# halajun/VDO_SLAM

Measured on AMD Instinct MI355X. Metric: frames/sec (per-frame hot path, KITTI-0000-shaped 1242x375) + ms/LM-iter (batch factor graph), higher is better.
Workload: dtype f64 (LM, RANSAC) / u8,i32,f32 (front-end, tracking)

## Files before the change

### include/vdo_slam_hip.h

```cpp
#ifndef VDO_SLAM_HIP_H_
#define VDO_SLAM_HIP_H_
#include <stdint.h>

#ifdef __cplusplus
extern "C" {
#endif

typedef enum vdo_status {
  VDO_OK = 0,
  VDO_ERR_INVALID = -1,
  VDO_ERR_NO_DEVICE = -2,
  VDO_ERR_OOM = -3,
  VDO_ERR_UNSUPPORTED = -4,
  VDO_ERR_INTERNAL = -5
} vdo_status;

int vdo_version(void);
const char* vdo_last_error(void);

typedef struct vdo_ctx vdo_ctx;
int vdo_ctx_create(int device, void* hip_stream, vdo_ctx** out);
int vdo_ctx_destroy(vdo_ctx* ctx);
int vdo_ctx_synchronize(vdo_ctx* ctx);
int vdo_ctx_stream(vdo_ctx* ctx, void** hip_stream_out);
// ... 174 lines not shown

typedef struct vdo_orb vdo_orb;
int vdo_orb_create(vdo_ctx* ctx, const vdo_orb_params* prm, int width, int height, vdo_orb** out);
int vdo_orb_destroy(vdo_orb* orb);
int vdo_orb_max_keypoints(const vdo_orb* orb, int* n);
int vdo_orb_extract(vdo_orb* orb, const uint8_t* gray, int stride, int src_is_device, vdo_keypoints* out);
int vdo_orb_extract_begin(vdo_orb* orb, const uint8_t* gray, int stride, int src_is_device);
int vdo_orb_extract_end(vdo_orb* orb, vdo_keypoints* out);
int vdo_orb_descriptors(vdo_orb* orb, uint8_t* desc32, int capacity_rows);
int vdo_orb_extract_desc(vdo_orb* orb, const uint8_t* gray, int stride, int src_is_device, vdo_keypoints* out, uint8_t* desc32);
int vdo_orb_level_info(vdo_orb* orb, int level, int* w, int* h, int* n_features, int* n_candidates);
int vdo_orb_get_pyramid(vdo_orb* orb, int level, uint8_t* out_bordered );
int vdo_orb_get_blurred(vdo_orb* orb, int level, uint8_t* out );
int vdo_orb_get_candidates(vdo_orb* orb, int level, float* x, float* y, float* response, float* angle, int cap, int* n);
int vdo_orb_last_timing(vdo_orb* orb, double ms[2]);
int vdo_orb_pyramid_launches(const vdo_orb* orb);

int vdo_depth_preprocess(vdo_ctx* ctx, float* depth, int64_t n, float bf, float depth_map_factor, int is_device);
int vdo_rgb2gray(vdo_ctx* ctx, const uint8_t* rgb, int64_t n_pixels, int channels, int rgb_order, uint8_t* gray);

typedef struct vdo_frame_images vdo_frame_images;
int vdo_frame_images_create(vdo_ctx* ctx, int width, int height, vdo_frame_images** out);
int vdo_frame_images_upload(vdo_frame_images* f, const float* depth, const float* flow, const int32_t* mask);
int vdo_frame_images_upload_on(vdo_ctx* ctx, vdo_frame_images* f, const float* depth, const float* flow, const int32_t* mask);
int vdo_frame_images_upload_device(vdo_frame_images* f, const float* depth_dev, const float* flow_dev, const int32_t* mask_dev);
int vdo_frame_images_depth_preprocess(vdo_frame_images* f, float bf, float depth_map_factor);
int vdo_frame_images_ingest_device(vdo_frame_images* f, const float* depth_dev, const float* flow_dev, const int32_t* mask_dev, float bf, float depth_map_factor,
                                   int convert_depth);
int vdo_frame_images_destroy(vdo_frame_images* f);
int vdo_frame_images_set_ctx(vdo_frame_images* f, vdo_ctx* ctx);
// ... 120 lines not shown
```

### vdo_slam_amd/csrc/orb.hip

```cpp
#include <algorithm>
#include <atomic>
#include <chrono>
#include <cmath>
#include <condition_variable>
#include <functional>
#include <memory>
#include <mutex>
#include <thread>
#include <cstring>
#include <vector>

#include "../../include/vdo_slam_hip.h"
#include "ctx.hpp"
#include "host_pool.hpp"
#include "orb_pattern.hpp"

namespace vdo {

constexpr int kEdge = 19, kHalfPatch = 15, kPatch = 31;
constexpr int kSpecCand = 24576;
constexpr int kMaxCellDim = 68;
static_assert(kMaxCellDim <= 128, "k_fast_cells packs cell-local coordinates in 7 bits");

struct LevelDesc { int w, h, bw, bh; int64_t off; int64_t off_inner; int64_t off_blur; };
struct CellDesc { int level, x0, y0, x1, y1, addx, addy, pad; };

__device__ __forceinline__ int reflect101(int p, int len) {
  if (len == 1) return 0;
  while (p < 0 || p >= len) { if (p < 0) p = -p; else p = 2 * (len - 1) - p; }
  return p;
}

__global__ void k_rgb2gray(const uint8_t* __restrict__ src, int64_t n, int ch, int rgb_order, uint8_t* __restrict__ dst) {
  const int64_t i = blockIdx.x * (int64_t)blockDim.x + threadIdx.x;
  if (i >= n) return;
// ... 142 lines not shown
  r[4] = c[3]; r[5] = c[-stride + 3]; r[6] = c[-2 * stride + 2]; r[7] = c[-3 * stride + 1];
  r[8] = c[-3 * stride]; r[9] = c[-3 * stride - 1]; r[10] = c[-2 * stride - 2]; r[11] = c[-stride - 3];
  r[12] = c[-3]; r[13] = c[stride - 3]; r[14] = c[2 * stride - 2]; r[15] = c[3 * stride - 1];
  int best = -1000;
#pragma unroll
  for (int s = 0; s < 16; ++s) {
    int mb = 1000, md = 1000;
#pragma unroll
    for (int k = 0; k < 9; ++k) { const int q = r[(s + k) & 15]; mb = min(mb, q - v); md = min(md, v - q); }
    best = max(best, max(mb, md));
  }
  return best > t ? best - 1 : 0;
}

__global__ __launch_bounds__(256) void k_fast_cells(const uint8_t* __restrict__ pyr, const LevelDesc* __restrict__ levels,
                                                    const CellDesc* __restrict__ cells, int ini_th, int min_th, int cell_cap,
                                                    int* __restrict__ out_cnt, uint32_t* __restrict__ out_pack) {
  __shared__ uint8_t roi[kMaxCellDim * kMaxCellDim];
  __shared__ uint8_t sc[kMaxCellDim * kMaxCellDim];
  __shared__ int s_wave[4], s_total;
  const CellDesc C = cells[blockIdx.x];
  const LevelDesc L = levels[C.level];
  const int w = C.x1 - C.x0, h = C.y1 - C.y0, tid = threadIdx.x;
  const uint8_t* img = pyr + L.off_inner;
  for (int i = tid; i < w * h; i += 256) { const int y = i / w, x = i - y * w; roi[y * kMaxCellDim + x] = img[(size_t)(C.y0 + y) * L.bw + (C.x0 + x)]; }
  __syncthreads();
  const int npix = w * h;
  const int per = (npix + 255) / 256;
  int t = ini_th;
  for (int pass = 0; pass < 2; ++pass) {
    for (int i = tid; i < npix; i += 256) {
      const int y = i / w, x = i - y * w;
      int s = 0;
      if (x >= 3 && x < w - 3 && y >= 3 && y < h - 3 && w >= 7 && h >= 7) s = fast_score_lds(roi, kMaxCellDim, x, y, t);
      sc[y * kMaxCellDim + x] = (uint8_t)s;
    }
// ... 14 lines not shown
    int incl = cnt;
#pragma unroll
    for (int off = 1; off < 64; off <<= 1) { const int v = __shfl_up(incl, off, 64); if (lane >= off) incl += v; }
    if (lane == 63) s_wave[wv] = incl;
    __syncthreads();
    if (tid == 0) { int a = 0; for (int q = 0; q < 4; ++q) { const int v = s_wave[q]; s_wave[q] = a; a += v; } s_total = a; }
    __syncthreads();
    const int total = s_total;
    if (total > 0 || pass == 1) {
      int pos = s_wave[wv] + incl - cnt;
      for (int k = 0; k < per; ++k) {
        if (!(keep & (1u << k))) continue;
        const int i = tid * per + k;
        const int y = i / w, x = i - y * w;
        if (pos < cell_cap)
          out_pack[(size_t)blockIdx.x * cell_cap + pos] = (uint32_t)x | ((uint32_t)y << 7) | ((uint32_t)sc[y * kMaxCellDim + x] << 24);
        ++pos;
      }
      if (tid == 0) out_cnt[blockIdx.x] = total;
      return;
    }
    t = min_th;
    __syncthreads();
  }
}

struct UMax { int v[kHalfPatch + 2]; };

__device__ __forceinline__ float fast_atan2_dev(float y, float x) {
  const float p1 = 0.9997878412794807f * (float)(180 / M_PI), p3 = -0.3258083974640975f * (float)(180 / M_PI);
  const float p5 = 0.1555786518463281f * (float)(180 / M_PI), p7 = -0.04432655554792128f * (float)(180 / M_PI);
  const float ax = fabsf(x), ay = fabsf(y);
  float a, c, c2;
  if (ax >= ay) { c = ay / (ax + (float)2.2204460492503131e-16); c2 = c * c; a = (((p7 * c2 + p5) * c2 + p3) * c2 + p1) * c; }
  else { c = ax / (ay + (float)2.2204460492503131e-16); c2 = c * c; a = 90.f - (((p7 * c2 + p5) * c2 + p3) * c2 + p1) * c; }
  if (x < 0) a = 180.f - a;
  if (y < 0) a = 360.f - a;
  return a;
}

__global__ __launch_bounds__(256) void k_compact_angle(const uint8_t* __restrict__ pyr, const LevelDesc* __restrict__ levels,
                                                       const CellDesc* __restrict__ cells, const int* __restrict__ cnt, const int* __restrict__ cell_level,
                                                       int* __restrict__ level_cnt, const uint32_t* __restrict__ pack, int ncells, int cell_cap, UMax um,
                                                       float* __restrict__ ox, float* __restrict__ oy, float* __restrict__ oresp,
                                                       float* __restrict__ oang, int* __restrict__ olevel) {
  const int cell = blockIdx.x;
  const int n = min(cnt[cell], cell_cap);
  const CellDesc C = cells[cell];
  const int lvl = C.level;
  const LevelDesc L = levels[lvl];
  const uint8_t* img = pyr + L.off_inner;
  const int lane = threadIdx.x & 63, wv = threadIdx.x >> 6;
  __shared__ int s_part[4], s_lvl[17];
// ... 7 lines not shown
    if (cell == 0 && threadIdx.x < 17) s_lvl[threadIdx.x] = 0;
    __syncthreads();
    base = s_part[0] + s_part[1] + s_part[2] + s_part[3];
    if (cell == 0) {
      int mx = 0;
      for (int c = threadIdx.x; c < ncells; c += 256) { const int r = cnt[c], v = min(r, cell_cap); if (v) atomicAdd(&s_lvl[cell_level[c]], v); mx = max(mx, r); }
      atomicMax(&s_lvl[16], mx);
      __syncthreads();
      if (threadIdx.x < 16) level_cnt[threadIdx.x] = s_lvl[threadIdx.x];
      if (threadIdx.x == 0) { int t = 0; for (int q = 0; q < 16; ++q) t += s_lvl[q]; level_cnt[16] = t; level_cnt[17] = s_lvl[16]; }
    }
  }
  for (int k = wv; k < n; k += 4) {
    const uint32_t pk = pack[(size_t)cell * cell_cap + k];
    const int x = (int)(pk & 0x7f) + C.addx, y = (int)((pk >> 7) & 0x7f) + C.addy, s = (int)(pk >> 24);
    const int cx = x + (kEdge - 3), cy = y + (kEdge - 3);
    int m10 = 0, m01 = 0;
    if (lane < 31) {
      const int v = lane - kHalfPatch;
      const int d = um.v[v < 0 ? -v : v];
      const uint8_t* row = img + (size_t)(cy + v) * L.bw + cx;
      int rs = 0;
      for (int u = -d; u <= d; ++u) { const int p = row[u]; m10 += u * p; rs += p; }
      m01 = v * rs;
    }
#pragma unroll
    for (int off = 32; off > 0; off >>= 1) { m10 += __shfl_down(m10, off, 64); m01 += __shfl_down(m01, off, 64); }
    if (lane == 0) {
      const int o = base + k;
      ox[o] = (float)x; oy[o] = (float)y; oresp[o] = (float)s; olevel[o] = lvl;
      oang[o] = fast_atan2_dev((float)m01, (float)m10);
    }
  }
}

struct Blur7 { int k[7]; };
struct OrbPattern { int4 q[64]; };

__device__ __forceinline__ void sincos_exact_dev(float angle, float* s_out, float* c_out) {
  const double x = (double)angle;
  const int k = (int)(x * 0.63661977236758138 + 0.5);
  const double r = (x - k * 1.57079632673412561417e+00) - k * 6.07710050650619224932e-11;
  const double z = r * r;
  const double sp = r * (1.0 + z * (-1.0 / 6 + z * (1.0 / 120 + z * (-1.0 / 5040 + z * (1.0 / 362880 + z * (-1.0 / 39916800 + z * (1.0 / 6227020800.0 +
                    z * (-1.0 / 1307674368000.0 + z * (1.0 / 355687428096000.0)))))))));
  const double cp = 1.0 + z * (-1.0 / 2 + z * (1.0 / 24 + z * (-1.0 / 720 + z * (1.0 / 40320 + z * (-1.0 / 3628800 + z * (1.0 / 479001600 +
                    z * (-1.0 / 87178291200.0 + z * (1.0 / 20922789888000.0))))))));
// ... 222 lines not shown
  std::vector<float> scale;
  UMax um{};
  Blur7 blur{};
  PyrDesc pyr{};
  PyrDesc pyr2{};
  std::vector<void*> allocs;
  uint8_t *d_src = nullptr, *d_pyr = nullptr, *d_blur = nullptr;
  LevelDesc* d_levels = nullptr; CellDesc* d_cells = nullptr; int* d_cell_level = nullptr;
  int *d_cnt = nullptr, *d_offs = nullptr, *d_level_cnt = nullptr; uint32_t* d_pack = nullptr;
  float *d_x = nullptr, *d_y = nullptr, *d_resp = nullptr, *d_ang = nullptr; int* d_lvl = nullptr;
  int64_t pyr_bytes = 0, blur_bytes = 0;
  int dense_cap = 0;
  std::vector<int> sel_dense;
  OrbPattern* d_pat = nullptr; int* d_sel = nullptr; uint8_t* d_desc = nullptr; int desc_cap = 0;
  float* h_pin = nullptr;
  float* h_over = nullptr; size_t h_over_n = 0;
  const float *hx = nullptr, *hy = nullptr, *hresp = nullptr, *hang = nullptr; std::vector<int> hlevel_cnt;
  int n_cand = 0;
  QuadTree qt[16];
  std::vector<int> sel[16];
  std::unique_ptr<LevelPool> pool;
  double ms_device = 0, ms_tree = 0;
  bool begun = false;
  hipEvent_t ev_cand = nullptr;
  std::chrono::steady_clock::time_point t_begin;
};

extern "C" int vdo_orb_pyramid_launches(const vdo_orb* o) {
  if (!o) return set_error(VDO_ERR_INVALID, "null handle");
  return o->pyr.n_levels ? (o->pyr2.lv1 > o->pyr2.lv0 ? 2 : 1) : (int)o->levels.size();
// ... 126 lines not shown
        for (int axis = 0; axis < 2; ++axis) {
          const int len = axis ? D->h[l] : D->w[l];
          for (int t0 = 0; t0 < len; t0 += 32) {
            int d0 = t0, d1 = std::min(t0 + 31, len - 1);
            for (int k = l; k > D->base; --k) {
              int s0, s1;
              src_range(d0, d1, axis ? D->sy[k] : D->sx[k], axis ? D->h[k - 1] : D->w[k - 1], axis == 1, s0, s1);
              d0 = s0; d1 = s1;
              worst = std::max(worst, d1 - d0 + 1);
            }
          }
        }
      }
    }
    if (worst > kPyrRegion) P.n_levels = 0;
  }
  {
    int* umax = o->um.v;
    int v, v0;
    const int vmax = (int)std::floor(kHalfPatch * std::sqrt(2.f) / 2 + 1);
    const int vmin = (int)std::ceil(kHalfPatch * std::sqrt(2.f) / 2);
    const double hp2 = kHalfPatch * kHalfPatch;
    for (v = 0; v <= vmax; ++v) umax[v] = (int)lrint(std::sqrt(hp2 - v * v));
    for (v = kHalfPatch, v0 = 0; v >= vmin; --v) { while (umax[v0] == umax[v0 + 1]) ++v0; umax[v] = v0; ++v0; }
  }
  {
    double kd[7], sum = 0;
    for (int i = 0; i < 7; ++i) { const double x = i - 3; kd[i] = std::exp(-0.5 / 4.0 * x * x); sum += kd[i]; }
    for (int i = 0; i < 7; ++i) o->blur.k[i] = (int)lrint((double)(float)(kd[i] / sum) * 256);
  }
  hipStream_t s = ctx->stream;
  auto dev = [&](size_t bytes) -> void* { void* p = nullptr; if (hipMalloc(&p, bytes ? bytes : 8) != hipSuccess) return nullptr; o->allocs.push_back(p); return p; };
  o->dense_cap = o->ncells * o->cell_cap;
  o->d_src = (uint8_t*)dev((size_t)w * h * 4);
  o->d_pyr = (uint8_t*)dev(o->pyr_bytes); o->d_blur = (uint8_t*)dev(o->blur_bytes);
  o->d_levels = (LevelDesc*)dev(sizeof(LevelDesc) * NL); o->d_cells = (CellDesc*)dev(sizeof(CellDesc) * o->ncells);
  o->d_cell_level = (int*)dev(4 * (size_t)o->ncells);
  o->d_pat = (OrbPattern*)dev(sizeof(OrbPattern));
  o->d_cnt = (int*)dev(4 * (size_t)o->ncells); o->d_offs = (int*)dev(4 * ((size_t)o->ncells + 1)); o->d_level_cnt = (int*)dev(4 * 32);
  o->d_pack = (uint32_t*)dev(4 * (size_t)o->dense_cap);
  o->d_x = (float*)dev(4 * (size_t)o->dense_cap * 5);
  if (o->d_x) {
    o->d_y = o->d_x + (size_t)o->dense_cap; o->d_resp = o->d_x + 2 * (size_t)o->dense_cap; o->d_ang = o->d_x + 3 * (size_t)o->dense_cap;
    o->d_lvl = (int*)(o->d_x + 4 * (size_t)o->dense_cap);
  }
  if (hipHostMalloc((void**)&o->h_pin, 4 * (32 + 5 * (size_t)kSpecCand)) != hipSuccess) o->h_pin = nullptr;
  for (void* p : o->allocs) if (!p) { vdo_orb_destroy(o); return set_error(VDO_ERR_OOM, "hipMalloc failed"); }
  if (!o->d_lvl || !o->h_pin) { vdo_orb_destroy(o); return set_error(VDO_ERR_OOM, "hipMalloc failed"); }
  hipMemcpyAsync(o->d_levels, o->levels.data(), sizeof(LevelDesc) * NL, hipMemcpyHostToDevice, s);
  hipMemcpyAsync(o->d_cells, o->cells.data(), sizeof(CellDesc) * o->ncells, hipMemcpyHostToDevice, s);
  hipMemcpyAsync(o->d_cell_level, o->cell_level.data(), 4 * (size_t)o->ncells, hipMemcpyHostToDevice, s);
  static_assert(sizeof(kOrbPattern31) == sizeof(OrbPattern), "256 tests x 4 signed bytes");
  hipMemcpyAsync(o->d_pat, kOrbPattern31, sizeof(OrbPattern), hipMemcpyHostToDevice, s);
  if (hipStreamSynchronize(s) != hipSuccess) { vdo_orb_destroy(o); return set_error(VDO_ERR_NO_DEVICE, "orb upload failed"); }
  if (hipEventCreateWithFlags(&o->ev_cand, hipEventDisableTiming) != hipSuccess) { vdo_orb_destroy(o); return set_error(VDO_ERR_NO_DEVICE, "hipEventCreate failed"); }
  {
    const char* e = std::getenv("VDO_ORB_THREADS");
    const int nw = e ? std::atoi(e) : 3;
    if (nw > 0) o->pool.reset(new LevelPool(std::min(nw, 15)));
  }
  *out = o;
// ... 10 lines not shown
      const LevelDesc& B = o->levels[o->pyr2.base];
      hipLaunchKernelGGL(k_pyramid_all, dim3(o->pyr2.tile_off[o->pyr2.n_levels]), dim3(256), 0, s, (const uint8_t*)(o->d_pyr + B.off_inner), B.bw, o->pyr2, (const LevelDesc*)o->d_levels, o->d_pyr);
    }
  } else {
    {
      const LevelDesc& L = o->levels[0];
      hipLaunchKernelGGL(k_border_copy, dim3((L.bw + 31) / 32, (L.bh + 7) / 8), tb, 0, s, gray_dev, L.w, L.h, stride, o->d_pyr + L.off, L.bw, L.bh);
    }
    for (int l = 1; l < NL; ++l) {
      const LevelDesc &P = o->levels[l - 1], &L = o->levels[l];
      const double sx = 1. / ((double)L.w / P.w), sy = 1. / ((double)L.h / P.h);
      hipLaunchKernelGGL(k_resize_border, dim3((L.bw + 31) / 32, (L.bh + 7) / 8), tb, 0, s, (const uint8_t*)(o->d_pyr + P.off_inner), P.w, P.h, P.bw,
                         o->d_pyr + L.off, L.w, L.h, sx, sy);
    }
  }
  hipLaunchKernelGGL(k_fast_cells, dim3(o->ncells), dim3(256), 0, s, (const uint8_t*)o->d_pyr, (const LevelDesc*)o->d_levels, (const CellDesc*)o->d_cells,
                     o->prm.ini_th, o->prm.min_th, o->cell_cap, o->d_cnt, o->d_pack);
  hipLaunchKernelGGL(k_compact_angle, dim3(o->ncells), dim3(256), 0, s, (const uint8_t*)o->d_pyr, (const LevelDesc*)o->d_levels, (const CellDesc*)o->d_cells,
                     (const int*)o->d_cnt, (const int*)o->d_cell_level, o->d_level_cnt, (const uint32_t*)o->d_pack, o->ncells, o->cell_cap, o->um, o->d_x, o->d_y, o->d_resp, o->d_ang, o->d_lvl);
  return VDO_OK;
}

static void orb_blur_stage(vdo_orb* o) {
  hipStream_t s = o->ctx->stream;
  BlurTiles bt{};
  int tot = 0;
  for (int l = 0; l < o->prm.n_levels; ++l) {
    const LevelDesc& L = o->levels[l];
    bt.off[l] = tot; bt.tiles_x[l] = (L.w + 31) / 32;
    tot += bt.tiles_x[l] * ((L.h + 31) / 32);
  }
  bt.off[o->prm.n_levels] = tot;
  hipLaunchKernelGGL(k_blur7_all, dim3(tot), dim3(256), 0, s, (const uint8_t*)o->d_pyr, (const LevelDesc*)o->d_levels, o->prm.n_levels, bt, o->blur, o->d_blur);
}

extern "C" int vdo_orb_extract_begin(vdo_orb* o, const uint8_t* gray, int stride, int src_is_device) {
  if (!o || !gray) return set_error(VDO_ERR_INVALID, "vdo_orb_extract_begin: null argument");
  int rc = ctx_bind(o->ctx);
  if (rc != VDO_OK) return rc;
  hipStream_t s = o->ctx->stream;
  const uint8_t* src = gray;
  int sstride = stride;
  if (!src_is_device) {
    if (stride == o->w) hipMemcpyAsync(o->d_src, gray, (size_t)o->w * o->h, hipMemcpyHostToDevice, s);
    else hipMemcpy2DAsync(o->d_src, o->w, gray, stride, o->w, o->h, hipMemcpyHostToDevice, s);
    src = o->d_src; sstride = o->w;
  }
  o->t_begin = std::chrono::steady_clock::now();
  orb_device_stage(o, src, sstride);
  int* hdr = (int*)o->h_pin;
  float* rows = o->h_pin + 32;
  const int spec = std::min(kSpecCand, o->dense_cap);
  hipMemcpyAsync(hdr, o->d_level_cnt, 4 * 32, hipMemcpyDeviceToHost, s);
  hipMemcpy2DAsync(rows, 4 * (size_t)spec, o->d_x, 4 * (size_t)o->dense_cap, 4 * (size_t)spec, 5, hipMemcpyDeviceToHost, s);
  hipEventRecord(o->ev_cand, s);
  orb_blur_stage(o);
  o->begun = true;
  return VDO_OK;
}

extern "C" int vdo_orb_extract(vdo_orb* o, const uint8_t* gray, int stride, int src_is_device, vdo_keypoints* out) {
  int rc = vdo_orb_extract_begin(o, gray, stride, src_is_device);
  return rc != VDO_OK ? rc : vdo_orb_extract_end(o, out);
}

extern "C" int vdo_orb_extract_end(vdo_orb* o, vdo_keypoints* out) {
  if (!o || !out) return set_error(VDO_ERR_INVALID, "vdo_orb_extract_end: null argument");
  if (!o->begun) return set_error(VDO_ERR_INVALID, "vdo_orb_extract_end without vdo_orb_extract_begin");
  o->begun = false;
  int rc = ctx_bind(o->ctx);
  if (rc != VDO_OK) return rc;
  hipStream_t s = o->ctx->stream;
  const auto t_begin = o->t_begin;
  int* hdr = (int*)o->h_pin;
  float* rows = o->h_pin + 32;
  const int spec = std::min(kSpecCand, o->dense_cap);
  if (hipEventSynchronize(o->ev_cand) != hipSuccess) return set_error(VDO_ERR_NO_DEVICE, "orb device stage failed: %s", hipGetErrorString(hipGetLastError()));
  if (hdr[17] > o->cell_cap) {
    o->hlevel_cnt.clear(); o->sel_dense.clear();
    return set_error(VDO_ERR_UNSUPPORTED, "vdo_orb_extract: a FAST cell has %d candidates, more than the %d kept per cell", hdr[17], o->cell_cap);
  }
  const int total = hdr[16];
  o->n_cand = total;
  o->hlevel_cnt.assign(hdr, hdr + 16);
  size_t pitch = (size_t)spec;
  if (total > spec) {
    if (o->h_over_n < (size_t)total) {
      if (o->h_over) hipHostFree(o->h_over);
      o->h_over = nullptr; o->h_over_n = 0;
      if (hipHostMalloc((void**)&o->h_over, 4 * 5 * (size_t)total) != hipSuccess) return set_error(VDO_ERR_OOM, "hipHostMalloc failed");
      o->h_over_n = (size_t)total;
    }
    hipMemcpy2DAsync(o->h_over, 4 * (size_t)total, o->d_x, 4 * (size_t)o->dense_cap, 4 * (size_t)total, 5, hipMemcpyDeviceToHost, s);
    if (hipStreamSynchronize(s) != hipSuccess) return set_error(VDO_ERR_NO_DEVICE, "orb D2H failed");
    rows = o->h_over; pitch = (size_t)total;
  }
  o->hx = rows; o->hy = rows + pitch; o->hresp = rows + 2 * pitch; o->hang = rows + 3 * pitch;
  const auto t_dev = std::chrono::steady_clock::now();
  const int NL = o->prm.n_levels;
  int lvl_pos[17];
  lvl_pos[0] = 0;
  for (int l = 0; l < NL; ++l) lvl_pos[l + 1] = lvl_pos[l] + o->hlevel_cnt[l];
  const int minB = kEdge - 3;
  auto level_task = [&](int l) {
    const LevelDesc& L = o->levels[l];
    const int pos = lvl_pos[l];
    o->qt[l].run(o->hx + pos, o->hy + pos, o->hresp + pos, o->hlevel_cnt[l], minB, L.w - kEdge + 3, minB, L.h - kEdge + 3, o->nfeat[l], o->sel[l]);
  };
  if (o->pool) o->pool->run(NL, level_task);
  else for (int l = 0; l < NL; ++l) level_task(l);
  int n = 0;
  o->sel_dense.clear();
  for (int l = 0; l < NL; ++l) {
    const int pos = lvl_pos[l];
    const float *cx = o->hx + pos, *cy = o->hy + pos, *cr = o->hresp + pos, *ca = o->hang + pos;
    const int patch = (int)(kPatch * o->scale[l]);
    for (int id : o->sel[l]) {
      o->sel_dense.push_back(pos + id);
      if (n >= out->capacity) return set_error(VDO_ERR_INVALID, "vdo_orb_extract: keypoint capacity %d too small", out->capacity);
      float x = cx[id] + minB, y = cy[id] + minB;
      if (l != 0) { x = x * o->scale[l]; y = y * o->scale[l]; }
      out->x[n] = x; out->y[n] = y; out->response[n] = cr[id]; out->angle[n] = ca[id];
      out->octave[n] = l; out->size[n] = (float)patch;
      ++n;
    }
  }
  out->n = n;
  const auto t_end = std::chrono::steady_clock::now();
  o->ms_device = std::chrono::duration<double, std::milli>(t_dev - t_begin).count();
  o->ms_tree = std::chrono::duration<double, std::milli>(t_end - t_dev).count();
  return VDO_OK;
}

extern "C" int vdo_orb_descriptors(vdo_orb* o, uint8_t* desc32, int capacity_rows) {
  if (!o || !desc32) return set_error(VDO_ERR_INVALID, "vdo_orb_descriptors: null argument");
  const int n = (int)o->sel_dense.size();
  if (n > capacity_rows) return set_error(VDO_ERR_INVALID, "vdo_orb_descriptors: %d keypoints, room for %d", n, capacity_rows);
  if (n == 0) return VDO_OK;
  int rc = ctx_bind(o->ctx);
  if (rc != VDO_OK) return rc;
  hipStream_t s = o->ctx->stream;
  if (n > o->desc_cap) {
    const int cap = std::max(n, 4096);
    int* ns = nullptr; uint8_t* nd = nullptr;
    if (hipMalloc((void**)&ns, 4 * (size_t)cap) != hipSuccess || hipMalloc((void**)&nd, 32 * (size_t)cap) != hipSuccess) { if (ns) hipFree(ns); return set_error(VDO_ERR_OOM, "hipMalloc failed"); }
// ... 11 lines not shown
  return VDO_OK;
}

extern "C" int vdo_orb_extract_desc(vdo_orb* o, const uint8_t* gray, int stride, int src_is_device, vdo_keypoints* out, uint8_t* desc32) {
  int rc = vdo_orb_extract(o, gray, stride, src_is_device, out);
  if (rc != VDO_OK || !desc32) return rc;
  return vdo_orb_descriptors(o, desc32, out->capacity);
}

extern "C" int vdo_orb_last_timing(vdo_orb* o, double ms[2]) {
  if (!o || !ms) return set_error(VDO_ERR_INVALID, "null argument");
  ms[0] = o->ms_device; ms[1] = o->ms_tree;
  return VDO_OK;
}

extern "C" int vdo_orb_level_info(vdo_orb* o, int level, int* w, int* h, int* n_features, int* n_candidates) {
  if (!o || level < 0 || level >= o->prm.n_levels) return set_error(VDO_ERR_INVALID, "bad level");
  if (w) *w = o->levels[level].w;
  if (h) *h = o->levels[level].h;
  if (n_features) *n_features = o->nfeat[level];
  if (n_candidates) *n_candidates = o->hlevel_cnt.empty() ? 0 : o->hlevel_cnt[level];
  return VDO_OK;
}

extern "C" int vdo_orb_get_pyramid(vdo_orb* o, int level, uint8_t* out_bordered) {
  if (!o || !out_bordered || level < 0 || level >= o->prm.n_levels) return set_error(VDO_ERR_INVALID, "bad argument");
  int rc = ctx_bind(o->ctx);
  if (rc != VDO_OK) return rc;
  const LevelDesc& L = o->levels[level];
  if (hipMemcpy(out_bordered, o->d_pyr + L.off, (size_t)L.bw * L.bh, hipMemcpyDeviceToHost) != hipSuccess) return set_error(VDO_ERR_NO_DEVICE, "D2H failed");
// ... 67 lines not shown
```

### vdo_slam_amd/frontend.py

```python
from __future__ import annotations

import ctypes as C

import numpy as np

from . import _capi as K


class OrbParamsC(C.Structure):
    _fields_ = [("n_features", C.c_int32), ("scale_factor", C.c_float), ("n_levels", C.c_int32),
                ("ini_th", C.c_int32), ("min_th", C.c_int32)]


class KeypointsC(C.Structure):
    _fields_ = [("capacity", C.c_int32), ("n", C.c_int32), ("x", K.c_float_p), ("y", K.c_float_p),
                ("response", K.c_float_p), ("angle", K.c_float_p), ("size", K.c_float_p), ("octave", K.c_int32_p)]


def _fp(a): return a.ctypes.data_as(K.c_float_p)
def _ip(a): return a.ctypes.data_as(K.c_int32_p)
def _u8(a): return a.ctypes.data_as(K.c_uint8_p)


_declared = False
# ... 76 lines not shown
            st = self._dev_out = (cap, a, octave, kp, C.byref(kp), _lib().vdo_orb_extract)
        _, a, octave, kp, kp_ref, fn = st
        K.check(fn(self._h, C.cast(C.c_void_p(gray_ptr), K.c_uint8_p), stride, 1, kp_ref))
        n = kp.n
        out = {k: v[:n] for k, v in a.items()}
        out["octave"] = octave[:n]
        return out

    def last_timing(self):
        ms = (C.c_double * 2)()
        L = _lib()
        L.vdo_orb_last_timing.argtypes = [C.c_void_p, C.POINTER(C.c_double)]
        K.check(L.vdo_orb_last_timing(self._h, ms))
        return ms[0], ms[1]

    def pyramid_launches(self):
        L = _lib()
        L.vdo_orb_pyramid_launches.argtypes = [C.c_void_p]
        return int(L.vdo_orb_pyramid_launches(self._h))

    def level_info(self, level):
        w, h, nf, nc = C.c_int(), C.c_int(), C.c_int(), C.c_int()
        K.check(_lib().vdo_orb_level_info(self._h, level, C.byref(w), C.byref(h), C.byref(nf), C.byref(nc)))
        return w.value, h.value, nf.value, nc.value

    def pyramid(self, level):
        w, h, _, _ = self.level_info(level)
        out = np.zeros((h + 38, w + 38), np.uint8)
        K.check(_lib().vdo_orb_get_pyramid(self._h, level, _u8(out)))
        return out
# ... 141 lines not shown
```

Baseline: 1388.

## Pipeline ORB per level group so host quadtrees overlap device FAST work

Splits pyramid construction, FAST detection and compaction into up to three level groups. Each group publishes its candidates straight into mapped pinned host memory along with a ticket word, and host worker threads spin on that word and start the per-level quadtree distribution as soon as their group is ready. Orientation is computed in a separate pass afterwards. The aim is to hide host quadtree time behind the remaining device work instead of waiting for the whole device stage to finish. In exchange it adds host busy-wait spinning, system-scope fences, extra small single-block launches, and a fallback path when candidate counts overflow.

```diff
diff --git a/include/vdo_slam_hip.h b/include/vdo_slam_hip.h
--- a/include/vdo_slam_hip.h
+++ b/include/vdo_slam_hip.h
@@ -212,6 +212,7 @@
 int vdo_orb_get_blurred(vdo_orb* orb, int level, uint8_t* out );
 int vdo_orb_get_candidates(vdo_orb* orb, int level, float* x, float* y, float* response, float* angle, int cap, int* n);
 int vdo_orb_last_timing(vdo_orb* orb, double ms[2]);
+int vdo_orb_last_level_timing(vdo_orb* orb, double group_ms[5], double level_ms[16]);
 int vdo_orb_pyramid_launches(const vdo_orb* orb);
 
 int vdo_depth_preprocess(vdo_ctx* ctx, float* depth, int64_t n, float bf, float depth_map_factor, int is_device);
diff --git a/vdo_slam_amd/csrc/orb.hip b/vdo_slam_amd/csrc/orb.hip
--- a/vdo_slam_amd/csrc/orb.hip
+++ b/vdo_slam_amd/csrc/orb.hip
@@ -19,6 +19,8 @@
 
 constexpr int kEdge = 19, kHalfPatch = 15, kPatch = 31;
 constexpr int kSpecCand = 24576;
+constexpr int kMaxGroups = 3;
+constexpr int kPinHdr = 32 + 32 * 4;
 constexpr int kMaxCellDim = 68;
 static_assert(kMaxCellDim <= 128, "k_fast_cells packs cell-local coordinates in 7 bits");
 
@@ -191,12 +193,13 @@
 }
 
 __global__ __launch_bounds__(256) void k_fast_cells(const uint8_t* __restrict__ pyr, const LevelDesc* __restrict__ levels,
-                                                    const CellDesc* __restrict__ cells, int ini_th, int min_th, int cell_cap,
+                                                    const CellDesc* __restrict__ cells, int cell0, int ini_th, int min_th, int cell_cap,
                                                     int* __restrict__ out_cnt, uint32_t* __restrict__ out_pack) {
   __shared__ uint8_t roi[kMaxCellDim * kMaxCellDim];
   __shared__ uint8_t sc[kMaxCellDim * kMaxCellDim];
   __shared__ int s_wave[4], s_total;
-  const CellDesc C = cells[blockIdx.x];
+  const int cell = cell0 + blockIdx.x;
+  const CellDesc C = cells[cell];
   const LevelDesc L = levels[C.level];
   const int w = C.x1 - C.x0, h = C.y1 - C.y0, tid = threadIdx.x;
   const uint8_t* img = pyr + L.off_inner;
@@ -241,10 +244,10 @@
         const int i = tid * per + k;
         const int y = i / w, x = i - y * w;
         if (pos < cell_cap)
-          out_pack[(size_t)blockIdx.x * cell_cap + pos] = (uint32_t)x | ((uint32_t)y << 7) | ((uint32_t)sc[y * kMaxCellDim + x] << 24);
+          out_pack[(size_t)cell * cell_cap + pos] = (uint32_t)x | ((uint32_t)y << 7) | ((uint32_t)sc[y * kMaxCellDim + x] << 24);
         ++pos;
       }
-      if (tid == 0) out_cnt[blockIdx.x] = total;
+      if (tid == 0) out_cnt[cell] = total;
       return;
     }
     t = min_th;
@@ -264,6 +267,21 @@
   if (x < 0) a = 180.f - a;
   if (y < 0) a = 360.f - a;
   return a;
+}
+
+__device__ __forceinline__ float ic_angle_wave(const uint8_t* __restrict__ img, int bw, int cx, int cy, int lane, const UMax& um) {
+  int m10 = 0, m01 = 0;
+  if (lane < 31) {
+    const int v = lane - kHalfPatch;
+    const int d = um.v[v < 0 ? -v : v];
+    const uint8_t* row = img + (size_t)(cy + v) * bw + cx;
+    int rs = 0;
+    for (int u = -d; u <= d; ++u) { const int p = row[u]; m10 += u * p; rs += p; }
+    m01 = v * rs;
+  }
+#pragma unroll
+  for (int off = 32; off > 0; off >>= 1) { m10 += __shfl_down(m10, off, 64); m01 += __shfl_down(m01, off, 64); }
+  return fast_atan2_dev((float)m01, (float)m10);
 }
 
 __global__ __launch_bounds__(256) void k_compact_angle(const uint8_t* __restrict__ pyr, const LevelDesc* __restrict__ levels,
@@ -301,23 +319,84 @@
   for (int k = wv; k < n; k += 4) {
     const uint32_t pk = pack[(size_t)cell * cell_cap + k];
     const int x = (int)(pk & 0x7f) + C.addx, y = (int)((pk >> 7) & 0x7f) + C.addy, s = (int)(pk >> 24);
-    const int cx = x + (kEdge - 3), cy = y + (kEdge - 3);
-    int m10 = 0, m01 = 0;
-    if (lane < 31) {
-      const int v = lane - kHalfPatch;
-      const int d = um.v[v < 0 ? -v : v];
-      const uint8_t* row = img + (size_t)(cy + v) * L.bw + cx;
-      int rs = 0;
-      for (int u = -d; u <= d; ++u) { const int p = row[u]; m10 += u * p; rs += p; }
-      m01 = v * rs;
-    }
-#pragma unroll
-    for (int off = 32; off > 0; off >>= 1) { m10 += __shfl_down(m10, off, 64); m01 += __shfl_down(m01, off, 64); }
+    const float ang = ic_angle_wave(img, L.bw, x + (kEdge - 3), y + (kEdge - 3), lane, um);
     if (lane == 0) {
       const int o = base + k;
       ox[o] = (float)x; oy[o] = (float)y; oresp[o] = (float)s; olevel[o] = lvl;
-      oang[o] = fast_atan2_dev((float)m01, (float)m10);
-    }
+      oang[o] = ang;
+    }
+  }
+}
+
+__global__ __launch_bounds__(256) void k_compact_group(const CellDesc* __restrict__ cells, const int* __restrict__ cnt, const uint32_t* __restrict__ pack, int c0, int cell_cap,
+                                                       int* __restrict__ cell_off, float* __restrict__ ox, float* __restrict__ oy, float* __restrict__ oresp, int* __restrict__ olevel) {
+  __shared__ int s_part[4];
+  const int cell = c0 + blockIdx.x;
+  const int lane = threadIdx.x & 63, wv = threadIdx.x >> 6;
+  int a = 0;
+  for (int c = threadIdx.x; c < cell; c += 256) a += min(cnt[c], cell_cap);
+#pragma unroll
+  for (int off = 32; off > 0; off >>= 1) a += __shfl_down(a, off, 64);
+  if (lane == 0) s_part[wv] = a;
+  __syncthreads();
+  const int base = s_part[0] + s_part[1] + s_part[2] + s_part[3];
+  const int n = min(cnt[cell], cell_cap);
+  const CellDesc C = cells[cell];
+  if (threadIdx.x == 0) cell_off[cell] = base;
+  for (int k = threadIdx.x; k < n; k += 256) {
+    const uint32_t pk = pack[(size_t)cell * cell_cap + k];
+    const int o = base + k;
+    ox[o] = (float)((int)(pk & 0x7f) + C.addx); oy[o] = (float)((int)((pk >> 7) & 0x7f) + C.addy); oresp[o] = (float)(int)(pk >> 24); olevel[o] = C.level;
+  }
+}
+
+constexpr int kPublishThreads = 1024;
+__global__ __launch_bounds__(kPublishThreads) void k_publish(const int* __restrict__ cnt, const int* __restrict__ cell_level, int c0, int c1, int cell_cap, int spec,
+                                                             const float* __restrict__ src, size_t spitch, int nrows, float* __restrict__ dst, size_t dpitch,
+                                                             int* __restrict__ hdr, uint32_t ticket) {
+  __shared__ int s_lvl[19];
+  const int tid = threadIdx.x;
+  if (tid < 19) s_lvl[tid] = 0;
+  __syncthreads();
+  int before = 0, tot = 0, mx = 0;
+  for (int c = tid; c < c1; c += kPublishThreads) {
+    const int r = cnt[c], v = min(r, cell_cap);
+    if (c < c0) before += v;
+    else { tot += v; if (v) atomicAdd(&s_lvl[cell_level[c]], v); mx = max(mx, r); }
+  }
+#pragma unroll
+  for (int off = 32; off > 0; off >>= 1) { before += __shfl_down(before, off, 64); tot += __shfl_down(tot, off, 64); mx = max(mx, __shfl_down(mx, off, 64)); }
+  if ((tid & 63) == 0) { atomicAdd(&s_lvl[18], before); atomicAdd(&s_lvl[16], tot); atomicMax(&s_lvl[17], mx); }
+  __syncthreads();
+  const int base = s_lvl[18], n = max(0, min(base + s_lvl[16], spec) - base);
+  if (tid < 18) hdr[tid] = tid == 16 ? base + s_lvl[16] : s_lvl[tid];
+  for (int e0 = tid; e0 < nrows * n; e0 += 8 * kPublishThreads) {
+    float v[8];
+#pragma unroll
+    for (int u = 0; u < 8; ++u) { const int e = e0 + u * kPublishThreads; if (e < nrows * n) { const int r = e / n, i = e - r * n; v[u] = src[r * spitch + base + i]; } }
+#pragma unroll
+    for (int u = 0; u < 8; ++u) { const int e = e0 + u * kPublishThreads; if (e < nrows * n) { const int r = e / n, i = e - r * n; dst[r * dpitch + base + i] = v[u]; } }
+  }
+  __threadfence_system();
+  __syncthreads();
+  if (tid == 0) *(volatile uint32_t*)(hdr + 18) = ticket;
+}
+
+__global__ __launch_bounds__(256) void k_angle_all(const uint8_t* __restrict__ pyr, const LevelDesc* __restrict__ levels, const CellDesc* __restrict__ cells,
+                                                   const int* __restrict__ cnt, const int* __restrict__ cell_off, const uint32_t* __restrict__ pack, int cell_cap, UMax um,
+                                                   float* __restrict__ oang) {
+  const int cell = blockIdx.x;
+  const int n = min(cnt[cell], cell_cap);
+  if (n == 0) return;
+  const CellDesc C = cells[cell];
+  const LevelDesc L = levels[C.level];
+  const uint8_t* img = pyr + L.off_inner;
+  const int lane = threadIdx.x & 63, wv = threadIdx.x >> 6, base = cell_off[cell];
+  for (int k = wv; k < n; k += 4) {
+    const uint32_t pk = pack[(size_t)cell * cell_cap + k];
+    const int x = (int)(pk & 0x7f) + C.addx, y = (int)((pk >> 7) & 0x7f) + C.addy;
+    const float ang = ic_angle_wave(img, L.bw, x + (kEdge - 3), y + (kEdge - 3), lane, um);
+    if (lane == 0) oang[base + k] = ang;
   }
 }
 
@@ -570,6 +649,13 @@
   std::vector<int> sel_dense;
   OrbPattern* d_pat = nullptr; int* d_sel = nullptr; uint8_t* d_desc = nullptr; int desc_cap = 0;
   float* h_pin = nullptr;
+  float* h_pin_dev = nullptr;
+  PyrDesc pyr1{};
+  int n_groups = 0, grp_lvl[kMaxGroups + 1] = {}, grp_cell[kMaxGroups + 1] = {};
+  uint32_t seq = 0;
+  bool piped = false;
+  const uint8_t* pend_gray = nullptr; int pend_stride = 0, pend_dev = 0;
+  double ms_group[kMaxGroups + 2] = {}, ms_level[16] = {};
   float* h_over = nullptr; size_t h_over_n = 0;
   const float *hx = nullptr, *hy = nullptr, *hresp = nullptr, *hang = nullptr; std::vector<int> hlevel_cnt;
   int n_cand = 0;
@@ -726,6 +812,21 @@
       }
     }
     if (worst > kPyrRegion) P.n_levels = 0;
+    if (P.n_levels) {
+      int* gl = o->grp_lvl;
+      gl[0] = 0; gl[1] = 1; o->n_groups = 1;
+      if (NL > 1) { gl[2] = split + 1; o->n_groups = 2; }
+      if (NL > split + 1) { gl[3] = NL; o->n_groups = 3; }
+      for (int g = 0; g <= o->n_groups; ++g)
+        o->grp_cell[g] = (int)(std::lower_bound(o->cell_level.begin(), o->cell_level.end(), gl[g]) - o->cell_level.begin());
+      PyrDesc& P1 = o->pyr1;
+      P1 = P;
+      P1.lv0 = 1;
+      int tot = 0;
+      for (int l = 0; l <= NL; ++l) P1.tile_off[l] = 0;
+      for (int l = P1.lv0; l < P1.lv1; ++l) { P1.tile_off[l] = tot; tot += P1.tiles_x[l] * ((P1.h[l] + 31) / 32); }
+      for (int l = std::max(P1.lv1, P1.lv0); l <= NL; ++l) P1.tile_off[l] = tot;
+    }
   }
   {
     int* umax = o->um.v;
@@ -756,7 +857,13 @@
     o->d_y = o->d_x + (size_t)o->dense_cap; o->d_resp = o->d_x + 2 * (size_t)o->dense_cap; o->d_ang = o->d_x + 3 * (size_t)o->dense_cap;
     o->d_lvl = (int*)(o->d_x + 4 * (size_t)o->dense_cap);
   }
-  if (hipHostMalloc((void**)&o->h_pin, 4 * (32 + 5 * (size_t)kSpecCand)) != hipSuccess) o->h_pin = nullptr;
+  if (hipHostMalloc((void**)&o->h_pin, 4 * (kPinHdr + 5 * (size_t)kSpecCand), hipHostMallocMapped) != hipSuccess) o->h_pin = nullptr;
+  if (o->h_pin) {
+    std::memset(o->h_pin, 0, 4 * (size_t)kPinHdr);
+    void* dp = nullptr;
+    if (hipHostGetDevicePointer(&dp, o->h_pin, 0) == hipSuccess) o->h_pin_dev = (float*)dp;
+    else { (void)hipGetLastError(); o->n_groups = 0; }
+  }
   for (void* p : o->allocs) if (!p) { vdo_orb_destroy(o); return set_error(VDO_ERR_OOM, "hipMalloc failed"); }
   if (!o->d_lvl || !o->h_pin) { vdo_orb_destroy(o); return set_error(VDO_ERR_OOM, "hipMalloc failed"); }
   hipMemcpyAsync(o->d_levels, o->levels.data(), sizeof(LevelDesc) * NL, hipMemcpyHostToDevice, s);
@@ -797,11 +904,43 @@
                          o->d_pyr + L.off, L.w, L.h, sx, sy);
     }
   }
-  hipLaunchKernelGGL(k_fast_cells, dim3(o->ncells), dim3(256), 0, s, (const uint8_t*)o->d_pyr, (const LevelDesc*)o->d_levels, (const CellDesc*)o->d_cells,
+  hipLaunchKernelGGL(k_fast_cells, dim3(o->ncells), dim3(256), 0, s, (const uint8_t*)o->d_pyr, (const LevelDesc*)o->d_levels, (const CellDesc*)o->d_cells, 0,
                      o->prm.ini_th, o->prm.min_th, o->cell_cap, o->d_cnt, o->d_pack);
   hipLaunchKernelGGL(k_compact_angle, dim3(o->ncells), dim3(256), 0, s, (const uint8_t*)o->d_pyr, (const LevelDesc*)o->d_levels, (const CellDesc*)o->d_cells,
                      (const int*)o->d_cnt, (const int*)o->d_cell_level, o->d_level_cnt, (const uint32_t*)o->d_pack, o->ncells, o->cell_cap, o->um, o->d_x, o->d_y, o->d_resp, o->d_ang, o->d_lvl);
   return VDO_OK;
+}
+
+static void orb_device_stage_groups(vdo_orb* o, const uint8_t* gray_dev, int stride) {
+  hipStream_t s = o->ctx->stream;
+  const int spec = std::min(kSpecCand, o->dense_cap);
+  int* ghdr = (int*)o->h_pin_dev + 32;
+  float* hrows = o->h_pin_dev + kPinHdr;
+  for (int g = 0; g < o->n_groups; ++g) {
+    if (g == 0) {
+      const LevelDesc& L = o->levels[0];
+      hipLaunchKernelGGL(k_border_copy, dim3((L.bw + 31) / 32, (L.bh + 7) / 8), dim3(32, 8), 0, s, gray_dev, L.w, L.h, stride, o->d_pyr + L.off, L.bw, L.bh);
+    } else if (g == 1) {
+      hipLaunchKernelGGL(k_pyramid_all, dim3(o->pyr1.tile_off[o->pyr1.n_levels]), dim3(256), 0, s, gray_dev, stride, o->pyr1, (const LevelDesc*)o->d_levels, o->d_pyr);
+    } else {
+      const LevelDesc& B = o->levels[o->pyr2.base];
+      hipLaunchKernelGGL(k_pyramid_all, dim3(o->pyr2.tile_off[o->pyr2.n_levels]), dim3(256), 0, s, (const uint8_t*)(o->d_pyr + B.off_inner), B.bw, o->pyr2, (const LevelDesc*)o->d_levels, o->d_pyr);
+    }
+    const int c0 = o->grp_cell[g], c1 = o->grp_cell[g + 1];
+    if (c1 > c0)
+      hipLaunchKernelGGL(k_fast_cells, dim3(c1 - c0), dim3(256), 0, s, (const uint8_t*)o->d_pyr, (const LevelDesc*)o->d_levels, (const CellDesc*)o->d_cells, c0,
+                         o->prm.ini_th, o->prm.min_th, o->cell_cap, o->d_cnt, o->d_pack);
+    if (c1 > c0)
+      hipLaunchKernelGGL(k_compact_group, dim3(c1 - c0), dim3(256), 0, s, (const CellDesc*)o->d_cells, (const int*)o->d_cnt, (const uint32_t*)o->d_pack, c0, o->cell_cap,
+                         o->d_offs, o->d_x, o->d_y, o->d_resp, o->d_lvl);
+    hipLaunchKernelGGL(k_publish, dim3(1), dim3(kPublishThreads), 0, s, (const int*)o->d_cnt, (const int*)o->d_cell_level, c0, c1, o->cell_cap, spec,
+                       (const float*)o->d_x, (size_t)o->dense_cap, 3, hrows, (size_t)spec, ghdr + 32 * g, o->seq);
+  }
+  if (o->ncells)
+    hipLaunchKernelGGL(k_angle_all, dim3(o->ncells), dim3(256), 0, s, (const uint8_t*)o->d_pyr, (const LevelDesc*)o->d_levels, (const CellDesc*)o->d_cells,
+                       (const int*)o->d_cnt, (const int*)o->d_offs, (const uint32_t*)o->d_pack, o->cell_cap, o->um, o->d_ang);
+  hipLaunchKernelGGL(k_publish, dim3(1), dim3(kPublishThreads), 0, s, (const int*)o->d_cnt, (const int*)o->d_cell_level, 0, o->ncells, o->cell_cap, spec,
+                     (const float*)o->d_ang, (size_t)o->dense_cap, 1, hrows + 3 * (size_t)spec, (size_t)spec, ghdr + 32 * kMaxGroups, o->seq);
 }
 
 static void orb_blur_stage(vdo_orb* o) {
@@ -817,10 +956,17 @@
   hipLaunchKernelGGL(k_blur7_all, dim3(tot), dim3(256), 0, s, (const uint8_t*)o->d_pyr, (const LevelDesc*)o->d_levels, o->prm.n_levels, bt, o->blur, o->d_blur);
 }
 
-extern "C" int vdo_orb_extract_begin(vdo_orb* o, const uint8_t* gray, int stride, int src_is_device) {
+static int orb_begin_prepare(vdo_orb* o, const uint8_t* gray) {
   if (!o || !gray) return set_error(VDO_ERR_INVALID, "vdo_orb_extract_begin: null argument");
   int rc = ctx_bind(o->ctx);
   if (rc != VDO_OK) return rc;
+  o->t_begin = std::chrono::steady_clock::now();
+  o->piped = o->n_groups > 0 && !std::getenv("VDO_ORB_NO_LEVEL_PIPELINE");
+  if (o->piped && ++o->seq == 0) ++o->seq;
+  return VDO_OK;
+}
+
+static void orb_begin_launch(vdo_orb* o, const uint8_t* gray, int stride, int src_is_device) {
   hipStream_t s = o->ctx->stream;
   const uint8_t* src = gray;
   int sstride = stride;
@@ -829,22 +975,89 @@
     else hipMemcpy2DAsync(o->d_src, o->w, gray, stride, o->w, o->h, hipMemcpyHostToDevice, s);
     src = o->d_src; sstride = o->w;
   }
-  o->t_begin = std::chrono::steady_clock::now();
-  orb_device_stage(o, src, sstride);
-  int* hdr = (int*)o->h_pin;
-  float* rows = o->h_pin + 32;
-  const int spec = std::min(kSpecCand, o->dense_cap);
-  hipMemcpyAsync(hdr, o->d_level_cnt, 4 * 32, hipMemcpyDeviceToHost, s);
-  hipMemcpy2DAsync(rows, 4 * (size_t)spec, o->d_x, 4 * (size_t)o->dense_cap, 4 * (size_t)spec, 5, hipMemcpyDeviceToHost, s);
+  if (o->piped) {
+    orb_device_stage_groups(o, src, sstride);
+  } else {
+    orb_device_stage(o, src, sstride);
+    int* hdr = (int*)o->h_pin;
+    float* rows = o->h_pin + kPinHdr;
+    const int spec = std::min(kSpecCand, o->dense_cap);
+    hipMemcpyAsync(hdr, o->d_level_cnt, 4 * 32, hipMemcpyDeviceToHost, s);
+    hipMemcpy2DAsync(rows, 4 * (size_t)spec, o->d_x, 4 * (size_t)o->dense_cap, 4 * (size_t)spec, 5, hipMemcpyDeviceToHost, s);
+  }
   hipEventRecord(o->ev_cand, s);
   orb_blur_stage(o);
+  o->ms_group[kMaxGroups + 1] = std::chrono::duration<double, std::milli>(std::chrono::steady_clock::now() - o->t_begin).count();
+}
+
+extern "C" int vdo_orb_extract_begin(vdo_orb* o, const uint8_t* gray, int stride, int src_is_device) {
+  int rc = orb_begin_prepare(o, gray);
+  if (rc != VDO_OK) return rc;
+  orb_begin_launch(o, gray, stride, src_is_device);
   o->begun = true;
   return VDO_OK;
 }
 
 extern "C" int vdo_orb_extract(vdo_orb* o, const uint8_t* gray, int stride, int src_is_device, vdo_keypoints* out) {
-  int rc = vdo_orb_extract_begin(o, gray, stride, src_is_device);
-  return rc != VDO_OK ? rc : vdo_orb_extract_end(o, out);
+  int rc = orb_begin_prepare(o, gray);
+  if (rc != VDO_OK) return rc;
+  if (o->piped && o->pool && out) { o->pend_gray = gray; o->pend_stride = stride; o->pend_dev = src_is_device; }
+  else orb_begin_launch(o, gray, stride, src_is_device);
+  o->begun = true;
+  return vdo_orb_extract_end(o, out);
+}
+
+static bool orb_trees_by_group(vdo_orb* o) {
+  const int NL = o->prm.n_levels, G = o->n_groups, spec = std::min(kSpecCand, o->dense_cap), minB = kEdge - 3;
+  const int* ghdr = (const int*)o->h_pin + 32;
+  const float* rows = o->h_pin + kPinHdr;
+  const auto t_begin = o->t_begin;
+  std::atomic<int> bad{0};
+  double seen[16];
+  auto wait_group = [&](int g) {
+    const int* hdr = ghdr + 32 * g;
+    volatile const uint32_t* word = (volatile const uint32_t*)(hdr + 18);
+    const auto t0 = std::chrono::steady_clock::now();
+    for (uint32_t spins = 0; *word != o->seq; ++spins) {
+      if (bad.load(std::memory_order_relaxed)) return false;
+      if ((spins & 1023u) == 1023u && std::chrono::duration<double, std::milli>(std::chrono::steady_clock::now() - t0).count() > 200.0) { bad.store(1); return false; }
+      __builtin_ia32_pause();
+    }
+    std::atomic_thread_fence(std::memory_order_acquire);
+    if (g < kMaxGroups && (hdr[17] > o->cell_cap || hdr[16] > spec)) { bad.store(1); return false; }
+    return true;
+  };
+  auto level_task = [&](int l) {
+    int g = 0;
+    while (l >= o->grp_lvl[g + 1]) ++g;
+    if (!wait_group(g)) return;
+    const auto t0 = std::chrono::steady_clock::now();
+    const int* hdr = ghdr + 32 * g;
+    int pos = hdr[16];
+    for (int k = o->grp_lvl[g + 1] - 1; k >= l; --k) pos -= hdr[k];
+    const LevelDesc& L = o->levels[l];
+    o->hlevel_cnt[l] = hdr[l];
+    o->qt[l].run(rows + pos, rows + spec + pos, rows + 2 * (size_t)spec + pos, hdr[l], minB, L.w - kEdge + 3, minB, L.h - kEdge + 3, o->nfeat[l], o->sel[l]);
+    const auto t1 = std::chrono::steady_clock::now();
+    seen[l] = std::chrono::duration<double, std::milli>(t0 - t_begin).count();
+    o->ms_level[l] = std::chrono::duration<double, std::milli>(t1 - t0).count();
+  };
+  for (int l = 0; l < 16; ++l) { seen[l] = 0; o->ms_level[l] = 0; }
+  o->hlevel_cnt.assign(16, 0);
+  auto mine = [&] {
+    if (o->pend_gray) { const uint8_t* g = o->pend_gray; o->pend_gray = nullptr; orb_begin_launch(o, g, o->pend_stride, o->pend_dev); }
+    level_task(0);
+  };
+  if (o->pool) o->pool->run_beside(NL - 1, [&](int i) { level_task(i + 1); }, mine);
+  else for (int l = 0; l < NL; ++l) level_task(l);
+  for (int g = 0; g < G; ++g) {
+    double m = 0;
+    for (int l = o->grp_lvl[g]; l < o->grp_lvl[g + 1]; ++l) if (seen[l] > 0 && (m == 0 || seen[l] < m)) m = seen[l];
+    o->ms_group[g] = m;
+  }
+  if (bad.load() || !wait_group(kMaxGroups)) return false;
+  o->ms_group[kMaxGroups] = std::chrono::duration<double, std::milli>(std::chrono::steady_clock::now() - t_begin).count();
+  return true;
 }
 
 extern "C" int vdo_orb_extract_end(vdo_orb* o, vdo_keypoints* out) {
@@ -852,13 +1065,26 @@
   if (!o->begun) return set_error(VDO_ERR_INVALID, "vdo_orb_extract_end without vdo_orb_extract_begin");
   o->begun = false;
   int rc = ctx_bind(o->ctx);
-  if (rc != VDO_OK) return rc;
+  if (rc != VDO_OK) { o->pend_gray = nullptr; return rc; }
   hipStream_t s = o->ctx->stream;
   const auto t_begin = o->t_begin;
+  const int NL = o->prm.n_levels;
   int* hdr = (int*)o->h_pin;
-  float* rows = o->h_pin + 32;
+  float* rows = o->h_pin + kPinHdr;
   const int spec = std::min(kSpecCand, o->dense_cap);
-  if (hipEventSynchronize(o->ev_cand) != hipSuccess) return set_error(VDO_ERR_NO_DEVICE, "orb device stage failed: %s", hipGetErrorString(hipGetLastError()));
+  int lvl_pos[17];
+  bool trees_done = false;
+  for (int g = 0; g <= kMaxGroups; ++g) o->ms_group[g] = 0;
+  if (o->piped) trees_done = orb_trees_by_group(o);
+  if (!trees_done && hipEventSynchronize(o->ev_cand) != hipSuccess) { o->hlevel_cnt.clear(); o->sel_dense.clear(); return set_error(VDO_ERR_NO_DEVICE, "orb device stage failed: %s", hipGetErrorString(hipGetLastError())); }
+  if (o->piped) {
+    const int* ghdr = (const int*)o->h_pin + 32;
+    for (int k = 0; k < 32; ++k) hdr[k] = 0;
+    for (int g = 0; g < o->n_groups; ++g) {
+      for (int l = o->grp_lvl[g]; l < o->grp_lvl[g + 1]; ++l) hdr[l] = ghdr[32 * g + l];
+      hdr[16] = ghdr[32 * g + 16]; hdr[17] = std::max(hdr[17], ghdr[32 * g + 17]);
+    }
+  }
   if (hdr[17] > o->cell_cap) {
     o->hlevel_cnt.clear(); o->sel_dense.clear();
     return set_error(VDO_ERR_UNSUPPORTED, "vdo_orb_extract: a FAST cell has %d candidates, more than the %d kept per cell", hdr[17], o->cell_cap);
@@ -868,6 +1094,7 @@
   o->hlevel_cnt.assign(hdr, hdr + 16);
   size_t pitch = (size_t)spec;
   if (total > spec) {
+    trees_done = false;
     if (o->h_over_n < (size_t)total) {
       if (o->h_over) hipHostFree(o->h_over);
       o->h_over = nullptr; o->h_over_n = 0;
@@ -880,19 +1107,22 @@
   }
   o->hx = rows; o->hy = rows + pitch; o->hresp = rows + 2 * pitch; o->hang = rows + 3 * pitch;
   const auto t_dev = std::chrono::steady_clock::now();
-  const int NL = o->prm.n_levels;
-  int lvl_pos[17];
   lvl_pos[0] = 0;
   for (int l = 0; l < NL; ++l) lvl_pos[l + 1] = lvl_pos[l] + o->hlevel_cnt[l];
+  if (!trees_done) {
+    const int minB = kEdge - 3;
+    auto level_task = [&](int l) {
+      const auto t0 = std::chrono::steady_clock::now();
+      const LevelDesc& L = o->levels[l];
+      const int pos = lvl_pos[l];
+      o->qt[l].run(o->hx + pos, o->hy + pos, o->hresp + pos, o->hlevel_cnt[l], minB, L.w - kEdge + 3, minB, L.h - kEdge + 3, o->nfeat[l], o->sel[l]);
+      o->ms_level[l] = std::chrono::duration<double, std::milli>(std::chrono::steady_clock::now() - t0).count();
+    };
+    if (o->pool) o->pool->run(NL, level_task);
+    else for (int l = 0; l < NL; ++l) level_task(l);
+  }
+  int n = 0;
   const int minB = kEdge - 3;
-  auto level_task = [&](int l) {
-    const LevelDesc& L = o->levels[l];
-    const int pos = lvl_pos[l];
-    o->qt[l].run(o->hx + pos, o->hy + pos, o->hresp + pos, o->hlevel_cnt[l], minB, L.w - kEdge + 3, minB, L.h - kEdge + 3, o->nfeat[l], o->sel[l]);
-  };
-  if (o->pool) o->pool->run(NL, level_task);
-  else for (int l = 0; l < NL; ++l) level_task(l);
-  int n = 0;
   o->sel_dense.clear();
   for (int l = 0; l < NL; ++l) {
     const int pos = lvl_pos[l];
@@ -910,8 +1140,8 @@
   }
   out->n = n;
   const auto t_end = std::chrono::steady_clock::now();
-  o->ms_device = std::chrono::duration<double, std::milli>(t_dev - t_begin).count();
-  o->ms_tree = std::chrono::duration<double, std::milli>(t_end - t_dev).count();
+  o->ms_device = trees_done && o->ms_group[0] > 0 ? o->ms_group[0] : std::chrono::duration<double, std::milli>(t_dev - t_begin).count();
+  o->ms_tree = std::chrono::duration<double, std::milli>(t_end - t_begin).count() - o->ms_device;
   return VDO_OK;
 }
 
@@ -953,6 +1183,13 @@
   return VDO_OK;
 }
 
+extern "C" int vdo_orb_last_level_timing(vdo_orb* o, double group_ms[5], double level_ms[16]) {
+  if (!o || !group_ms || !level_ms) return set_error(VDO_ERR_INVALID, "null argument");
+  for (int g = 0; g < kMaxGroups + 2; ++g) group_ms[g] = o->ms_group[g];
+  for (int l = 0; l < 16; ++l) level_ms[l] = l < o->prm.n_levels ? o->ms_level[l] : 0;
+  return VDO_OK;
+}
+
 extern "C" int vdo_orb_level_info(vdo_orb* o, int level, int* w, int* h, int* n_features, int* n_candidates) {
   if (!o || level < 0 || level >= o->prm.n_levels) return set_error(VDO_ERR_INVALID, "bad level");
   if (w) *w = o->levels[level].w;
diff --git a/vdo_slam_amd/frontend.py b/vdo_slam_amd/frontend.py
--- a/vdo_slam_amd/frontend.py
+++ b/vdo_slam_amd/frontend.py
@@ -114,6 +114,34 @@
         K.check(L.vdo_orb_last_timing(self._h, ms))
         return ms[0], ms[1]
 
+    def last_level_timing(self):
+        g, l = (C.c_double * 5)(), (C.c_double * 16)()
+        L = _lib()
+        L.vdo_orb_last_level_timing.argtypes = [C.c_void_p, C.POINTER(C.c_double), C.POINTER(C.c_double)]
+        K.check(L.vdo_orb_last_level_timing(self._h, g, l))
+        return list(g), list(l)[:self.nlevels]
+
+    def begin(self, gray: np.ndarray):
+        gray = np.ascontiguousarray(gray, dtype=np.uint8)
+        if gray.shape != (self.h, self.w):
+            raise ValueError(f"image {gray.shape}, extractor {(self.h, self.w)}")
+        L = _lib()
+        L.vdo_orb_extract_begin.argtypes = [C.c_void_p, K.c_uint8_p, C.c_int, C.c_int]
+        self._begin_src = gray
+        K.check(L.vdo_orb_extract_begin(self._h, _u8(gray), self.w, 0))
+
+    def end(self, capacity=None):
+        cap = capacity or self.max_keypoints
+        a = {k: np.zeros(cap, np.float32) for k in ("x", "y", "response", "angle", "size")}
+        octave = np.zeros(cap, np.int32)
+        kp = KeypointsC(cap, 0, _fp(a["x"]), _fp(a["y"]), _fp(a["response"]), _fp(a["angle"]), _fp(a["size"]), _ip(octave))
+        L = _lib()
+        L.vdo_orb_extract_end.argtypes = [C.c_void_p, C.POINTER(KeypointsC)]
+        K.check(L.vdo_orb_extract_end(self._h, C.byref(kp)))
+        out = {k: v[:kp.n].copy() for k, v in a.items()}
+        out["octave"] = octave[:kp.n].copy()
+        return out
+
     def pyramid_launches(self):
         L = _lib()
         L.vdo_orb_pyramid_launches.argtypes = [C.c_void_p]
```

Result: no change. 1391 (median of 3 runs) (+0.2%).
